# pps-lab/rofl-project-code

Measured on NVIDIA B200. Metric: range-proved commitment elements/s (prove & verify), higher is better.
Workload: dtype u32 (8 saturated 32-bit limbs of GF(2^255-19), IMAD.WIDE.U32 with 64-bit accumulate; scalars mod l)

## Files before the change

### rofl-project-code_b200/csrc/engine.cuh

```cuda
#pragma once
#include "kernels.cuh"
#include "rt.cuh"
#include <map>
#include <mutex>
#include <shared_mutex>
#include <condition_variable>
#include <thread>
#include <atomic>
#ifndef ROFL_EMUL
#include <sys/resource.h>
#endif
#include <algorithm>
#include <chrono>
#include <cstdio>

enum { ROFL_ERR_BITSIZE_ = -7 };
enum { DOM_RANGE_PROVE = 1, DOM_RANGE_VERIFY = 2, DOM_SQUARE = 3, DOM_L2_PROVE = 4, DOM_L2_VERIFY = 5, DOM_CRP = 6, DOM_RND_VEC = 7, DOM_RANDPROOF = 8, DOM_SQUARE_RAND = 9,
       DOM_CRP_BATCH = 0x62707263 ,
       DOM_SQ_RLC = 0x6c727173 ,
       DOM_RP_RLC = 0x6c727072 ,
       DOM_SRP_RLC = 0x6c727273  };
enum { PROF_FOLD = 0, PROF_MSM = 1, PROF_COMMIT = 2, PROF_SQUARE = 3, PROF_RTMSM = 4, PROF_TAIL = 5, PROF_FRZ = 6, PROF_SLOTS = 8 };

struct gens_entry { int n = 0; int cap = 0; niels_st *G = nullptr, *H = nullptr;
// ... 161 lines not shown
static inline void engine_destroy(rofl_engine &e) {
    for (lane *l : e.lanes) { for (int g = 0; g < ROFL_MAX_GROUPS; g++) { rt_sync(l->q[g].hi); rt_sync(l->q[g].lo); rt_sync(l->side[g]); } lane_delete(l); }
    e.lanes.clear();
    for (auto &pp : e.pins) rt_host_free(pp.first);
    e.pins.clear();
    std::lock_guard<std::mutex> lk(g_shared_mu);
    dev_shared *sh = e.sh; e.sh = nullptr;
    if (!sh || --sh->refs > 0) return;
    rt_raw_free(sh->tabB); rt_raw_free(sh->tabH);
    for (auto &g : sh->gens) { rt_raw_free(g.second.G); rt_raw_free(g.second.H); rt_raw_free(g.second.RTG); rt_raw_free(g.second.RTH); }
    for (auto &b : sh->bsgs) { rt_raw_free(b.second.keys); rt_raw_free(b.second.vals); }
    g_shared.erase(sh->device); delete sh;
    rt_trim();
}
static inline gens_entry engine_gens(rofl_engine &e, tables_use &tu, cudaStream_t s, int n, int m) {
    dev_shared &sh = *e.sh;
    for (;;) {
        auto it = sh.gens.find(n);
        if (it != sh.gens.end() && it->second.cap >= m) return it->second;
        tu.upgrade();
        gens_entry &g = sh.gens[n];
        if (g.cap >= m) continue;
        int newcap = std::max(m, g.cap * 2);
        niels_st *G = (niels_st *)rt_raw_malloc(sizeof(niels_st) * (size_t)n * newcap);
        niels_st *H = (niels_st *)rt_raw_malloc(sizeof(niels_st) * (size_t)n * newcap);
        if (g.cap) { rt_d2d(G, g.G, sizeof(niels_st) * (size_t)n * g.cap, s); rt_d2d(H, g.H, sizeof(niels_st) * (size_t)n * g.cap, s); }
        int cnt = 2 * (newcap - g.cap);
        LAUNCH(k_gens_build, dim3((cnt + 63) / 64), dim3(64), s, G, H, n, g.cap, newcap);
        rt_sync(s);
        rt_raw_free(g.G); rt_raw_free(g.H);
        g.n = n; g.cap = newcap; g.G = G; g.H = H;
    }
}
static inline void rt_fill(rt_tables &t, int c) { t.c = c; t.nw = msm_nw(c); t.B = 1 << (c - 1); msm_recode_const(t.K, c); }
static inline size_t rt_table_bytes(size_t cnt, int c) { return 2 * cnt * (size_t)msm_nw(c) * ((size_t)1 << (c - 1)) * sizeof(niels_st); }
static inline bool engine_rt(rofl_engine &e, tables_use &tu, cudaStream_t s, int n, int m, rt_tables &out) {
    if (!e.use_rt) return false;
    dev_shared &sh = *e.sh;
    for (;;) {
        gens_entry &g = sh.gens[n];
        if (g.rt_cap >= m) { g.last_use = ++sh.clock; out.G = g.RTG; out.H = g.RTH; rt_fill(out, g.rt_c); return true; }
        if (g.rt_nofit && m >= g.rt_nofit) return false;
        if (!tu.excl) { tu.upgrade(); continue; }
        const size_t cnt = (size_t)n * m;
        if ((double)rt_table_bytes(cnt, 8) > 170e9) { g.rt_nofit = m; return false; }
        rt_sync(s); rt_raw_free(g.RTG); rt_raw_free(g.RTH); g.RTG = g.RTH = nullptr; g.rt_cap = 0; g.rt_bytes = 0;
        rt_trim();
        const int want = std::max(8, std::min(RT_MAX_BITS, e.rt_bits));
        int c = 0;
        for (;;) {
            const size_t have = rt_free_mem();
            for (c = want; c >= 8; c--) if ((double)(rt_table_bytes(cnt, c) + cnt * msm_nw(c) * sizeof(p3_st)) <= e.rt_mem_frac * (double)have) break;
            if (c == want) break;
            gens_entry *victim = nullptr;
            for (auto &kv : sh.gens) if (&kv.second != &g && kv.second.RTG && (!victim || kv.second.last_use < victim->last_use)) victim = &kv.second;
            if (!victim) break;
            rt_raw_free(victim->RTG); rt_raw_free(victim->RTH); victim->RTG = victim->RTH = nullptr; victim->rt_cap = 0; victim->rt_bytes = 0;
        }
        if (c < 8) { g.rt_nofit = m; sh.free_hint = rt_free_mem(); return false; }
        rt_tables t; rt_fill(t, c);
        const size_t bytes = cnt * rt_row_entries(t) * sizeof(niels_st);
        niels_st *RTG = (niels_st *)rt_raw_malloc(bytes), *RTH = (niels_st *)rt_raw_malloc(bytes);
        {
            dev_buf P(cnt * t.nw * sizeof(p3_st), s);
            const size_t rows = cnt * t.nw, thr = rows * (t.B / 16);
            for (int which = 0; which < 2; which++) {
                LAUNCH(k_rt_shifts, dim3((unsigned)((cnt + 127) / 128)), dim3(128), s, P.as<p3_st>(), which ? g.H : g.G, (uint32_t)cnt, t.c, t.nw);
                LAUNCH(k_rt_rows, dim3((unsigned)((thr + 127) / 128)), dim3(128), s, which ? RTH : RTG, P.as<p3_st>(), rows, t.B);
            }
            rt_sync(s);
        }
        g.RTG = RTG; g.RTH = RTH; g.rt_cap = m; g.rt_c = c; g.rt_bytes = 2 * bytes;
        rt_trim();
        sh.free_hint = rt_free_mem();
    }
}
static inline void engine_drop_rt(rofl_engine &e) {
    std::unique_lock<std::shared_mutex> ex(e.sh->tab_mu);
    for (auto &g : e.sh->gens) { rt_raw_free(g.second.RTG); rt_raw_free(g.second.RTH); g.second.RTG = g.second.RTH = nullptr; g.second.rt_cap = 0; g.second.rt_bytes = 0; g.second.rt_nofit = 0; }
}
static inline int rt_blocks(size_t T, int C, int per_max = 0) {
    const size_t slots = 148 * RTM_BLOCKS, max_nb = std::max<size_t>(1, (T + 127) / 128);
    if (per_max > 0) {
        const size_t nb = std::min(max_nb, (T + 128 * (size_t)per_max - 1) / (128 * (size_t)per_max));
        return (int)std::max<size_t>(1, nb);
// ... 17 lines not shown
struct msm_plan { int c, nw; uint32_t slices, slice_len; bool big = false; uint32_t parts = 1; size_t out_count(size_t n_msm) const { return n_msm * slices * (size_t)nw; } };
static inline int msm_pick_c(size_t T) {
    int best = 8; double bc = 1e300;
    for (int c = 3; c <= 8; c++) { const double B = (double)(1 << (c - 1)), cost = (double)msm_nw(c) * ((double)T + B * c); if (cost < bc) { bc = cost; best = c; } }
    return best;
}
static inline size_t bm_min_terms() { static const size_t v = getenv("ROFL_BM_MIN") ? (size_t)atoll(getenv("ROFL_BM_MIN")) : (size_t)32768; return v; }
static inline msm_plan msm_plan_forced(size_t T, int c, int knob) {
    msm_plan p; p.c = std::max(3, std::min(16, c)); p.nw = msm_nw(p.c); p.slices = 1; p.slice_len = (uint32_t)T;
    if (p.c > 8) { p.big = true; p.parts = (uint32_t)std::max(1, std::min(8, knob)); return p; }
    if (T > 0) { p.slices = (uint32_t)std::max<size_t>(1, std::min<size_t>(std::max(knob, 1), T)); p.slice_len = (uint32_t)((T + p.slices - 1) / p.slices); p.slices = (uint32_t)((T + p.slice_len - 1) / p.slice_len); }
    return p;
}
static inline msm_plan msm_plan_for(size_t T, size_t n_msm, size_t big_min = 0) {
    msm_plan p; p.c = msm_pick_c(T); p.slices = 1; p.slice_len = (uint32_t)T;
    if (const char *fc = getenv("ROFL_MSM_C"))
        return msm_plan_forced(T, atoi(fc), getenv("ROFL_MSM_SLICES") ? atoi(getenv("ROFL_MSM_SLICES")) : 1);
    if (T >= (big_min ? big_min : bm_min_terms())) {
        p.big = true; p.c = std::max(9, std::min(16, ilog2_sz(T + 1) - 6)); p.nw = msm_nw(p.c);
        const size_t threads = n_msm * (size_t)p.nw * ((size_t)1 << (p.c - 1));
        p.parts = (uint32_t)std::max<size_t>(1, std::min<size_t>(8, (148 * 1024 + threads - 1) / threads));
        return p;
    }
    const size_t wpb = MSM_THREADS >> (p.c - 1), blocks = n_msm * ((msm_nw(p.c) + wpb - 1) / wpb), slots = 148 * 4;
    if (blocks < slots && T >= 4096) {
        p.slices = (uint32_t)std::min<size_t>((slots + blocks - 1) / blocks, T / 2048);
        p.slice_len = (uint32_t)((T + p.slices - 1) / p.slices); p.slices = (uint32_t)((T + p.slice_len - 1) / p.slice_len);
        p.c = msm_pick_c(p.slice_len);
    }
    p.nw = msm_nw(p.c);
    return p;
}
static inline void run_msm(rofl_engine &e, cudaStream_t s, msm_args a, const msm_plan &p, uint32_t n_msm) {
    a.c = p.c; a.nw = p.nw; a.slices = p.slices; a.slice_len = p.slice_len; msm_recode_const(a.K, p.c);
    void *tk = rt_prof_begin(PROF_MSM, s);
    if (p.big) {
        const size_t B = (size_t)1 << (p.c - 1), nslot = (size_t)n_msm * p.nw * (B + 1);
        dev_buf d_start(4 * nslot, s), d_cur(4 * nslot, s), d_sorted(4 * (size_t)n_msm * p.nw * a.T, s), d_bkt(sizeof(p3_st) * (size_t)n_msm * p.nw * B * p.parts, s);
        a.bm_start = d_start.as<uint32_t>(); a.bm_cur = d_cur.as<uint32_t>(); a.bm_sorted = d_sorted.as<uint32_t>(); a.bm_bkt = d_bkt.as<p3_st>(); a.parts = p.parts;
        a.top_bits = (uint32_t)(254 - p.c * (p.nw - 1)); a.parts_top = 0;
        if ((int)a.top_bits < p.c - 4) a.parts_top = (uint32_t)((B * p.parts) >> (a.top_bits + 1));
        rt_memset(d_start.p, 0, 4 * nslot, s);
        const dim3 gt((unsigned)((a.T + 255) / 256), n_msm);
        LAUNCH(k_bm_hist, gt, dim3(256), s, a, 0);
        LAUNCH_COOP(k_bm_scan, dim3(p.nw, n_msm), dim3(256), s, a);
        LAUNCH(k_bm_hist, gt, dim3(256), s, a, 1);
        LAUNCH(k_bm_accum, dim3((unsigned)(((size_t)p.nw * B * p.parts + 127) / 128), n_msm), dim3(128), s, a);
        LAUNCH_COOP(k_bm_reduce, dim3(p.nw, n_msm), dim3(128), s, a);
    } else {
        const int wpb = MSM_THREADS >> (p.c - 1);
        LAUNCH_COOP(k_msm, dim3((p.nw + wpb - 1) / wpb, n_msm, p.slices), dim3(MSM_THREADS), s, a);
    }
    rt_prof_end(PROF_MSM, tk, s);
}
static inline msm_seg mk_seg(const void *base, uint32_t count, uint32_t stride, int kind, uint32_t np = 0, int hi = 0) { msm_seg s; s.base = base; s.count = count; s.stride = stride; s.kind = kind; s.np = np; s.hi = hi; return s; }
static inline void run_finalize(cudaStream_t s, const finalize_args &f) { LAUNCH_COOP(k_finalize, dim3(f.count), dim3(FIN_THREADS), s, f); }
static inline void fin_windows(finalize_args &f, const p3_st *win, const msm_plan &p) { f.windows = win; f.c = p.c; f.nw = p.nw; f.slices = p.slices; }


static void absorb_commitments(rofl_engine &e, cudaStream_t s, transcript *d_ts, const uint8_t *d_V32, int label_id, int n, int m, int C) {
    if (m <= e.ts_host_m) {
        ts_absorb_args aa = {}; aa.ts = d_ts; aa.V32 = d_V32; aa.m = (uint32_t)m; aa.n = (uint32_t)n; aa.label_id = label_id;
        LAUNCH_COOP(k_ts_absorbV, dim3(C), dim3(TS_THREADS), s, aa);
        return;
    }
    std::vector<uint8_t> hV(32 * (size_t)C * m); std::vector<transcript> ts(C);
    rt_d2h(hV.data(), d_V32, hV.size(), s); rt_sync(s);
// ... 1022 lines not shown
```

### rofl-project-code_b200/csrc/fe25519.cuh

```cuda
#pragma once
#include <stdint.h>
#include <string.h>

#if defined(__CUDACC__)
#define HD __host__ __device__ __forceinline__
#define HDNI static __host__ __device__ __noinline__
#else
#define HD inline
#define HDNI static inline
#endif
#define FE_ASSERT(c) ((void)0)
#ifndef FE_MUL_ROWS
#define FE_MUL_ROWS 1
#endif
#ifndef FE_INLINE_MUL
#define FE_INLINE_MUL 1
#endif
#if defined(__CUDACC__) && !FE_INLINE_MUL
#define HDMUL static __host__ __device__ __noinline__
#elif defined(__CUDACC__)
#define HDMUL __host__ __device__ __forceinline__
#else
#define HDMUL inline
#endif

#if !defined(__CUDACC__)
struct alignas(16) uint4 { uint32_t x, y, z, w; };
static inline uint4 make_uint4(uint32_t x, uint32_t y, uint32_t z, uint32_t w) { uint4 r; r.x = x; r.y = y; r.z = z; r.w = w; return r; }
#define __align__(n) alignas(n)
#endif

#define FE_LIMBS 8
struct fe { uint32_t v[8]; };

HD void fe_0(fe &h) { for (int i = 0; i < 8; i++) h.v[i] = 0; }
HD void fe_1(fe &h) { fe_0(h); h.v[0] = 1; }
HD void fe_carry(fe &h, const fe &f) { h = f; }

HD void fe_add(fe &h, const fe &f, const fe &g) {
#if defined(__CUDA_ARCH__)
    uint32_t r0, r1, r2, r3, r4, r5, r6, r7, c;
    asm("add.cc.u32 %0, %9, %17;\n\taddc.cc.u32 %1, %10, %18;\n\taddc.cc.u32 %2, %11, %19;\n\taddc.cc.u32 %3, %12, %20;\n\t"
        "addc.cc.u32 %4, %13, %21;\n\taddc.cc.u32 %5, %14, %22;\n\taddc.cc.u32 %6, %15, %23;\n\taddc.cc.u32 %7, %16, %24;\n\taddc.u32 %8, 0, 0;"
        : "=&r"(r0), "=&r"(r1), "=&r"(r2), "=&r"(r3), "=&r"(r4), "=&r"(r5), "=&r"(r6), "=&r"(r7), "=&r"(c)
        : "r"(f.v[0]), "r"(f.v[1]), "r"(f.v[2]), "r"(f.v[3]), "r"(f.v[4]), "r"(f.v[5]), "r"(f.v[6]), "r"(f.v[7]),
          "r"(g.v[0]), "r"(g.v[1]), "r"(g.v[2]), "r"(g.v[3]), "r"(g.v[4]), "r"(g.v[5]), "r"(g.v[6]), "r"(g.v[7]));
    c *= 38;
    asm("add.cc.u32 %0, %0, %8;\n\taddc.cc.u32 %1, %1, 0;\n\taddc.cc.u32 %2, %2, 0;\n\taddc.cc.u32 %3, %3, 0;\n\t"
        "addc.cc.u32 %4, %4, 0;\n\taddc.cc.u32 %5, %5, 0;\n\taddc.cc.u32 %6, %6, 0;\n\taddc.cc.u32 %7, %7, 0;\n\taddc.u32 %8, 0, 0;"
        : "+r"(r0), "+r"(r1), "+r"(r2), "+r"(r3), "+r"(r4), "+r"(r5), "+r"(r6), "+r"(r7), "+r"(c));
    r0 += 38 * c;
    h.v[0] = r0; h.v[1] = r1; h.v[2] = r2; h.v[3] = r3; h.v[4] = r4; h.v[5] = r5; h.v[6] = r6; h.v[7] = r7;
#else
    uint64_t c = 0; uint32_t r[8];
    for (int i = 0; i < 8; i++) { c += (uint64_t)f.v[i] + g.v[i]; r[i] = (uint32_t)c; c >>= 32; }
    c *= 38;
    for (int i = 0; i < 8; i++) { c += r[i]; r[i] = (uint32_t)c; c >>= 32; }
    r[0] += 38 * (uint32_t)c;
    for (int i = 0; i < 8; i++) h.v[i] = r[i];
#endif
}
HD void fe_sub(fe &h, const fe &f, const fe &g) {
#if defined(__CUDA_ARCH__)
    uint32_t r0, r1, r2, r3, r4, r5, r6, r7, b;
    asm("sub.cc.u32 %0, %9, %17;\n\tsubc.cc.u32 %1, %10, %18;\n\tsubc.cc.u32 %2, %11, %19;\n\tsubc.cc.u32 %3, %12, %20;\n\t"
        "subc.cc.u32 %4, %13, %21;\n\tsubc.cc.u32 %5, %14, %22;\n\tsubc.cc.u32 %6, %15, %23;\n\tsubc.cc.u32 %7, %16, %24;\n\tsubc.u32 %8, 0, 0;"
        : "=&r"(r0), "=&r"(r1), "=&r"(r2), "=&r"(r3), "=&r"(r4), "=&r"(r5), "=&r"(r6), "=&r"(r7), "=&r"(b)
        : "r"(f.v[0]), "r"(f.v[1]), "r"(f.v[2]), "r"(f.v[3]), "r"(f.v[4]), "r"(f.v[5]), "r"(f.v[6]), "r"(f.v[7]),
          "r"(g.v[0]), "r"(g.v[1]), "r"(g.v[2]), "r"(g.v[3]), "r"(g.v[4]), "r"(g.v[5]), "r"(g.v[6]), "r"(g.v[7]));
    b = (b & 1) * 38;
    asm("sub.cc.u32 %0, %0, %8;\n\tsubc.cc.u32 %1, %1, 0;\n\tsubc.cc.u32 %2, %2, 0;\n\tsubc.cc.u32 %3, %3, 0;\n\t"
        "subc.cc.u32 %4, %4, 0;\n\tsubc.cc.u32 %5, %5, 0;\n\tsubc.cc.u32 %6, %6, 0;\n\tsubc.cc.u32 %7, %7, 0;\n\tsubc.u32 %8, 0, 0;"
        : "+r"(r0), "+r"(r1), "+r"(r2), "+r"(r3), "+r"(r4), "+r"(r5), "+r"(r6), "+r"(r7), "+r"(b));
    r0 -= 38 * (b & 1);
    h.v[0] = r0; h.v[1] = r1; h.v[2] = r2; h.v[3] = r3; h.v[4] = r4; h.v[5] = r5; h.v[6] = r6; h.v[7] = r7;
#else
    int64_t c = 0; uint32_t r[8];
    for (int i = 0; i < 8; i++) { c += (int64_t)f.v[i] - (int64_t)g.v[i]; r[i] = (uint32_t)c; c >>= 32; }
    c *= 38;
    for (int i = 0; i < 8; i++) { c += r[i]; r[i] = (uint32_t)c; c >>= 32; }
    r[0] -= 38 * (uint32_t)(-c);
    for (int i = 0; i < 8; i++) h.v[i] = r[i];
#endif
}
HD void fe_sub4(fe &h, const fe &f, const fe &g) { fe_sub(h, f, g); }
HD void fe_neg(fe &h, const fe &f) { fe z; fe_0(z); fe_sub(h, z, f); }

#if defined(__CUDA_ARCH__)
__device__ __forceinline__ uint64_t fe_mad_wide(uint32_t a, uint32_t b, uint32_t c) {
    uint64_t d; asm("mad.wide.u32 %0, %1, %2, %3;" : "=l"(d) : "r"(a), "r"(b), "l"((uint64_t)c)); return d;
}
__device__ __forceinline__ void fe_reduce512(fe &h, const uint32_t t[16]) {
    uint64_t d0 = fe_mad_wide(t[8], 38, t[0]), d1 = fe_mad_wide(t[9], 38, t[1]), d2 = fe_mad_wide(t[10], 38, t[2]), d3 = fe_mad_wide(t[11], 38, t[3]);
    uint64_t d4 = fe_mad_wide(t[12], 38, t[4]), d5 = fe_mad_wide(t[13], 38, t[5]), d6 = fe_mad_wide(t[14], 38, t[6]), d7 = fe_mad_wide(t[15], 38, t[7]);
    uint32_t r0 = (uint32_t)d0, r1, r2, r3, r4, r5, r6, r7, top;
    asm("add.cc.u32 %0, %8, %9;\n\taddc.cc.u32 %1, %10, %11;\n\taddc.cc.u32 %2, %12, %13;\n\taddc.cc.u32 %3, %14, %15;\n\t"
        "addc.cc.u32 %4, %16, %17;\n\taddc.cc.u32 %5, %18, %19;\n\taddc.cc.u32 %6, %20, %21;\n\taddc.u32 %7, %22, 0;"
        : "=&r"(r1), "=&r"(r2), "=&r"(r3), "=&r"(r4), "=&r"(r5), "=&r"(r6), "=&r"(r7), "=&r"(top)
        : "r"((uint32_t)d1), "r"((uint32_t)(d0 >> 32)), "r"((uint32_t)d2), "r"((uint32_t)(d1 >> 32)), "r"((uint32_t)d3), "r"((uint32_t)(d2 >> 32)),
          "r"((uint32_t)d4), "r"((uint32_t)(d3 >> 32)), "r"((uint32_t)d5), "r"((uint32_t)(d4 >> 32)), "r"((uint32_t)d6), "r"((uint32_t)(d5 >> 32)),
          "r"((uint32_t)d7), "r"((uint32_t)(d6 >> 32)), "r"((uint32_t)(d7 >> 32)));
    uint32_t c = top * 38;
    asm("add.cc.u32 %0, %0, %8;\n\taddc.cc.u32 %1, %1, 0;\n\taddc.cc.u32 %2, %2, 0;\n\taddc.cc.u32 %3, %3, 0;\n\t"
        "addc.cc.u32 %4, %4, 0;\n\taddc.cc.u32 %5, %5, 0;\n\taddc.cc.u32 %6, %6, 0;\n\taddc.cc.u32 %7, %7, 0;\n\taddc.u32 %8, 0, 0;"
        : "+r"(r0), "+r"(r1), "+r"(r2), "+r"(r3), "+r"(r4), "+r"(r5), "+r"(r6), "+r"(r7), "+r"(c));
    r0 += 38 * c;
    h.v[0] = r0; h.v[1] = r1; h.v[2] = r2; h.v[3] = r3; h.v[4] = r4; h.v[5] = r5; h.v[6] = r6; h.v[7] = r7;
}
#define FE_MAC(lo, hi, ex, a, b) asm("mad.lo.cc.u32 %0, %3, %4, %0;\n\tmadc.hi.cc.u32 %1, %3, %4, %1;\n\taddc.u32 %2, %2, 0;" : "+r"(lo), "+r"(hi), "+r"(ex) : "r"(a), "r"(b))
#define FE_MUL0(lo, hi, a, b) do { uint64_t p_; asm("mul.wide.u32 %0, %1, %2;" : "=l"(p_) : "r"(a), "r"(b)); lo = (uint32_t)p_; hi = (uint32_t)(p_ >> 32); } while (0)
__device__ __forceinline__ void fe_columns_to_words(uint32_t t[16], const uint32_t lo[15], const uint32_t hi[15], const uint32_t ex[15]) {
    t[0] = lo[0];
    asm("add.cc.u32 %0, %15, %30;\n\taddc.cc.u32 %1, %16, %31;\n\taddc.cc.u32 %2, %17, %32;\n\taddc.cc.u32 %3, %18, %33;\n\taddc.cc.u32 %4, %19, %34;\n\t"
        "addc.cc.u32 %5, %20, %35;\n\taddc.cc.u32 %6, %21, %36;\n\taddc.cc.u32 %7, %22, %37;\n\taddc.cc.u32 %8, %23, %38;\n\taddc.cc.u32 %9, %24, %39;\n\t"
        "addc.cc.u32 %10, %25, %40;\n\taddc.cc.u32 %11, %26, %41;\n\taddc.cc.u32 %12, %27, %42;\n\taddc.cc.u32 %13, %28, %43;\n\taddc.u32 %14, %29, 0;"
        : "=&r"(t[1]), "=&r"(t[2]), "=&r"(t[3]), "=&r"(t[4]), "=&r"(t[5]), "=&r"(t[6]), "=&r"(t[7]), "=&r"(t[8]), "=&r"(t[9]), "=&r"(t[10]), "=&r"(t[11]), "=&r"(t[12]), "=&r"(t[13]), "=&r"(t[14]), "=&r"(t[15])
        : "r"(lo[1]), "r"(lo[2]), "r"(lo[3]), "r"(lo[4]), "r"(lo[5]), "r"(lo[6]), "r"(lo[7]), "r"(lo[8]), "r"(lo[9]), "r"(lo[10]), "r"(lo[11]), "r"(lo[12]), "r"(lo[13]), "r"(lo[14]), "r"(hi[14]),
          "r"(hi[0]), "r"(hi[1]), "r"(hi[2]), "r"(hi[3]), "r"(hi[4]), "r"(hi[5]), "r"(hi[6]), "r"(hi[7]), "r"(hi[8]), "r"(hi[9]), "r"(hi[10]), "r"(hi[11]), "r"(hi[12]), "r"(hi[13]));
    asm("add.cc.u32 %0, %0, %14;\n\taddc.cc.u32 %1, %1, %15;\n\taddc.cc.u32 %2, %2, %16;\n\taddc.cc.u32 %3, %3, %17;\n\taddc.cc.u32 %4, %4, %18;\n\t"
        "addc.cc.u32 %5, %5, %19;\n\taddc.cc.u32 %6, %6, %20;\n\taddc.cc.u32 %7, %7, %21;\n\taddc.cc.u32 %8, %8, %22;\n\taddc.cc.u32 %9, %9, %23;\n\t"
        "addc.cc.u32 %10, %10, %24;\n\taddc.cc.u32 %11, %11, %25;\n\taddc.cc.u32 %12, %12, %26;\n\taddc.u32 %13, %13, %27;"
        : "+r"(t[2]), "+r"(t[3]), "+r"(t[4]), "+r"(t[5]), "+r"(t[6]), "+r"(t[7]), "+r"(t[8]), "+r"(t[9]), "+r"(t[10]), "+r"(t[11]), "+r"(t[12]), "+r"(t[13]), "+r"(t[14]), "+r"(t[15])
        : "r"(ex[0]), "r"(ex[1]), "r"(ex[2]), "r"(ex[3]), "r"(ex[4]), "r"(ex[5]), "r"(ex[6]), "r"(ex[7]), "r"(ex[8]), "r"(ex[9]), "r"(ex[10]), "r"(ex[11]), "r"(ex[12]), "r"(ex[13]));
}
__device__ __forceinline__ void fe_mul_rows(uint32_t t[16], const fe &f, const fe &g) {
    uint32_t e[16], o[17];
    for (int k = 0; k < 16; k++) e[k] = 0;
    for (int k = 0; k < 17; k++) o[k] = 0;
    FE_MUL0(e[0], e[1], f.v[0], g.v[0]);
    FE_MUL0(e[2], e[3], f.v[0], g.v[2]);
    FE_MUL0(e[4], e[5], f.v[0], g.v[4]);
    FE_MUL0(e[6], e[7], f.v[0], g.v[6]);
    FE_MUL0(o[1], o[2], f.v[0], g.v[1]);
    FE_MUL0(o[3], o[4], f.v[0], g.v[3]);
    FE_MUL0(o[5], o[6], f.v[0], g.v[5]);
    FE_MUL0(o[7], o[8], f.v[0], g.v[7]);
    asm("mad.lo.cc.u32 %0, %8, %9, %0;\n\tmadc.hi.cc.u32 %1, %8, %9, %1;\n\tmadc.lo.cc.u32 %2, %8, %10, %2;\n\tmadc.hi.cc.u32 %3, %8, %10, %3;\n\tmadc.lo.cc.u32 %4, %8, %11, %4;\n\tmadc.hi.cc.u32 %5, %8, %11, %5;\n\tmadc.lo.cc.u32 %6, %8, %12, %6;\n\tmadc.hi.u32 %7, %8, %12, %7;"
        : "+r"(e[2]), "+r"(e[3]), "+r"(e[4]), "+r"(e[5]), "+r"(e[6]), "+r"(e[7]), "+r"(e[8]), "+r"(e[9])
        : "r"(f.v[1]), "r"(g.v[1]), "r"(g.v[3]), "r"(g.v[5]), "r"(g.v[7]));
    asm("mad.lo.cc.u32 %0, %9, %10, %0;\n\tmadc.hi.cc.u32 %1, %9, %10, %1;\n\tmadc.lo.cc.u32 %2, %9, %11, %2;\n\tmadc.hi.cc.u32 %3, %9, %11, %3;\n\tmadc.lo.cc.u32 %4, %9, %12, %4;\n\tmadc.hi.cc.u32 %5, %9, %12, %5;\n\tmadc.lo.cc.u32 %6, %9, %13, %6;\n\tmadc.hi.cc.u32 %7, %9, %13, %7;\n\taddc.u32 %8, 0, 0;"
        : "+r"(o[1]), "+r"(o[2]), "+r"(o[3]), "+r"(o[4]), "+r"(o[5]), "+r"(o[6]), "+r"(o[7]), "+r"(o[8]), "+r"(o[9])
// ... 215 lines not shown
```

### rofl-project-code_b200/csrc/kernels.cuh

```cuda
#pragma once
#include "devfn.cuh"

#include "rt.cuh"
#ifndef ROFL_EMUL
#define KERNEL extern "C" __global__
#define LB(t, b) __launch_bounds__(t, b)
#define DEV __device__ __forceinline__
#define KLAUNCH(k, coop, PARAMS, ARGS) void launch_##k(dim3 g_, dim3 b_, cudaStream_t s_, KL_UNPACK PARAMS) { rt_host_timer t_(&rt_host_prof::launch, #k); void *tl_ = rt_timeline_begin(#k, s_, g_.x * g_.y * g_.z); k<<<g_, b_, 0, s_>>> ARGS; rt_check(cudaGetLastError(), #k); rt_timeline_end(tl_, s_); rt_count_launch(#k); }
#else
#define KERNEL static
#define LB(t, b)
#define DEV inline
#define KLAUNCH(k, coop, PARAMS, ARGS) void launch_##k(dim3 g_, dim3 b_, cudaStream_t s_, KL_UNPACK PARAMS) { (void)s_; emu_launch(g_, b_, coop, [&] { k ARGS; }); }
#endif
#define KL_UNPACK(...) __VA_ARGS__
#if defined(KG_ALL)
#define KG_TABLES 1
#define KG_COMMIT 1
#define KG_SCALAR 1
#define KG_MSM 1
#define KG_FOLD 1
#define KG_SQUARE 1
#define KG_BSGS 1
#define KG_TS 1
// ... 218 lines not shown

#ifdef KG_MSM
KERNEL void LB(128, 2) k_bits_sum(p3_st *partial, const uint64_t *vals, const niels_st *G, const niels_st *H, int n, int m) {
    __shared__ p3_st buf[128];
    int c = blockIdx.y, tid = threadIdx.x;
    size_t N = (size_t)n * m;
    ge_p3 acc; ge_p3_0(acc);
    for (size_t k = (size_t)blockIdx.x * blockDim.x + tid; k < N; k += (size_t)gridDim.x * blockDim.x) {
        size_t j = k / n; int i = (int)(k % n);
        bool bit = (vals[(size_t)c * m + j] >> i) & 1;
        acc_add_niels(acc, (bit ? G : H) + k, !bit);
    }
    block_sum_p3(acc, buf, tid, blockDim.x);
    if (tid == 0) st_p3(partial + (size_t)c * gridDim.x + blockIdx.x, acc);
}
KLAUNCH(k_bits_sum, true, (p3_st *partial, const uint64_t *vals, const niels_st *G, const niels_st *H, int n, int m), (partial, vals, G, H, n, m))
#endif

#define MSM_THREADS 128
#define MSM_SORT 8192
#define MSM_MAXW 85
struct msm_seg { const void *base; uint32_t count; uint32_t stride; int kind; uint32_t np; int hi; };
struct msm_var { const sc_st *scalars; msm_seg seg[4]; };
struct msm_args {
    msm_var v[2]; uint32_t split;
    int nseg; uint32_t T, scalar_stride;
    int c, nw; uint32_t K[9];
    uint32_t slices, slice_len;
    p3_st *out;
    uint32_t *bm_start, *bm_cur, *bm_sorted; p3_st *bm_bkt; uint32_t parts;
    uint32_t top_bits, parts_top;
};
HD int msm_nw(int c) { return (254 + c - 1) / c; }
HD void msm_recode_const(uint32_t K[9], int c) {
    for (int i = 0; i < 9; i++) K[i] = 0;
    const uint32_t bm1 = (1u << (c - 1)) - 1; const int nw = msm_nw(c);
    for (int w = 0; w < nw; w++) { int bit = c * w; uint64_t v = (uint64_t)bm1 << (bit & 31); K[bit >> 5] |= (uint32_t)v; if ((bit >> 5) + 1 < 9) K[(bit >> 5) + 1] |= (uint32_t)(v >> 32); }
}
HD void msm_recode(uint32_t xk[9], const sc &x, const uint32_t K[9]) {
    uint64_t cy = 0;
    for (int i = 0; i < 8; i++) { cy += (uint64_t)x.v[i] + K[i]; xk[i] = (uint32_t)cy; cy >>= 32; }
    xk[8] = (uint32_t)cy + K[8];
}
HD int msm_digit(const uint32_t xk[9], int w, int c) {
    int bit = c * w, i = bit >> 5, sh = bit & 31;
    uint64_t v = (uint64_t)xk[i] | ((uint64_t)(i + 1 < 9 ? xk[i + 1] : 0) << 32);
    return (int)((v >> sh) & ((1u << c) - 1)) - ((1 << (c - 1)) - 1);
}
HD void msm_add_term(ge_p3 &acc, const msm_var &v, int nseg, uint32_t idx, uint32_t t, bool neg) {
    uint32_t start = 0; const void *base = nullptr; size_t rec = 0; int kind = -1;
    for (int s = 0; s < nseg; s++) {
        const msm_seg &g = v.seg[s];
        const bool here = kind < 0 && t < start + g.count;
        if (here) { const uint32_t q = t - start, j = g.np ? (q / g.np) * 2 * g.np + (g.hi ? g.np : 0) + q % g.np : q; base = g.base; rec = (size_t)idx * g.stride + j; kind = g.kind; }
        start += g.count;
    }
    if (kind == 0) acc_add_niels(acc, (const niels_st *)base + rec, neg);
    else if (kind == 1) acc_add_p3(acc, (const p3_st *)base + rec, neg);
}
#ifdef KG_MSM
KERNEL void LB(MSM_THREADS, 4) k_msm(msm_args a) {
    __shared__ uint16_t sorted[MSM_SORT];
    __shared__ int cnt[MSM_THREADS], off[MSM_THREADS + 1], cur[MSM_THREADS];
    __shared__ p3_st bk[MSM_THREADS];
    const int tid = threadIdx.x, c = a.c, B = 1 << (c - 1), wpb = MSM_THREADS / B;
    const int w0 = blockIdx.x * wpb, wl_mine = tid / B, b_mine = tid & (B - 1);
    const uint32_t msm = blockIdx.y, slice = blockIdx.z;
    const msm_var &v = msm < a.split ? a.v[0] : a.v[1];
    const uint32_t idx = msm < a.split ? msm : msm - a.split;
// ... 875 lines not shown
void launch_k_ipp_fold_points(dim3 g_, dim3 b_, cudaStream_t s_, fold_args a);
void launch_k_decompress_batch(dim3 g_, dim3 b_, cudaStream_t s_, p3_st *out, uint8_t *out32, const uint8_t *in, size_t D, size_t Dp, size_t K, const p3_st *offset, int *bad);
void launch_k_decompress(dim3 g_, dim3 b_, cudaStream_t s_, p3_st *out, uint8_t *out32, const uint8_t *in, size_t count_in, size_t count_out, const p3_st *offset, int *bad, size_t bad_group);
void launch_k_verify_tables(dim3 g_, dim3 b_, cudaStream_t s_, sc_st *tab, vtab_layout t, sc_st *var, uint32_t var_stride, const sc_st *chal, int chal_stride, const sc_st *yinvpow2, const sc_st *zpow2, int m);
void launch_k_verify_scalars(dim3 g_, dim3 b_, cudaStream_t s_, sc_st *gh, const sc_st *tab, vtab_layout t, const sc_st *chal, int chal_stride, int n, int C);
void launch_k_square_prove(dim3 g_, dim3 b_, cudaStream_t s_, square_args a);
void launch_k_sigma_prove(dim3 g_, dim3 b_, cudaStream_t s_, sigma_args a);
void launch_k_sigma_verify(dim3 g_, dim3 b_, cudaStream_t s_, int kind, const uint8_t *proofs, const uint8_t *commits, size_t D, const niels_st *tabB, const niels_st *tabH, int *result, size_t group);
void launch_k_sigma_rlc_prep(dim3 g_, dim3 b_, cudaStream_t s_, sigma_rlc_args a);
void launch_k_sigma_rlc_scalars(dim3 g_, dim3 b_, cudaStream_t s_, sigma_rlc_args a);
void launch_k_sigma_rlc_points(dim3 g_, dim3 b_, cudaStream_t s_, sigma_rlc_args a);
void launch_k_square_verify(dim3 g_, dim3 b_, cudaStream_t s_, const uint8_t *proofs, const uint8_t *commits, size_t D, const niels_st *tabB, const niels_st *tabH, int *result, size_t group);
void launch_k_hash_tree(dim3 g_, dim3 b_, cudaStream_t s_, uint8_t *out, const uint8_t *in, size_t n);
void launch_k_aggregate(dim3 g_, dim3 b_, cudaStream_t s_, uint8_t *out, const uint8_t *pts, size_t n_clients, size_t D, int init_base, int *bad);
void launch_k_bsgs_build(dim3 g_, dim3 b_, cudaStream_t s_, unsigned long long *keys, uint32_t *vals, uint32_t cap, uint32_t m, const niels_st *tabB, int *distinct);
void launch_k_bsgs_solve(dim3 g_, dim3 b_, cudaStream_t s_, uint8_t *out_sc, float *out_f32, const uint8_t *pts, size_t D, const unsigned long long *keys, const uint32_t *vals, uint32_t cap, uint32_t m, uint64_t size, uint64_t max_it, int bsgs_bits, int n_bits, int frac, const niels_st *tabB, int *flags);
void launch_k_f32_to_scalar(dim3 g_, dim3 b_, cudaStream_t s_, uint8_t *out, const float *v, size_t D, int n_bits, int frac, int *flags);
void launch_k_scalar_to_f32(dim3 g_, dim3 b_, cudaStream_t s_, float *out, const uint8_t *in, size_t D, int n_bits, int frac);
void launch_k_l2_sums(dim3 g_, dim3 b_, cudaStream_t s_, sc_st *partial, const float *v, const uint8_t *blind, size_t D, int n_bits, int frac, int *flags);
void launch_k_join96(dim3 g_, dim3 b_, cudaStream_t s_, uint8_t *out96, const uint8_t *pairs64, const uint8_t *sq64, size_t D);
void launch_k_validate_points(dim3 g_, dim3 b_, cudaStream_t s_, const uint8_t *rec, size_t stride, size_t offset, size_t D, int *bad, size_t group);
void launch_k_split96(dim3 g_, dim3 b_, cudaStream_t s_, uint8_t *L, uint8_t *sq64, uint8_t *csq, const uint8_t *in96, size_t D);
void launch_k_points_sum(dim3 g_, dim3 b_, cudaStream_t s_, p3_st *partial, const uint8_t *pts32, size_t D, int *bad);
void launch_k_crp_sums(dim3 g_, dim3 b_, cudaStream_t s_, sc_st *partial, const float *v, const uint8_t *blind, size_t D, int n_bits, int frac, pow_tab ctab, int *flags);
void launch_k_crp_pows(dim3 g_, dim3 b_, cudaStream_t s_, sc_st *out, size_t D, pow_tab ctab);
void launch_k_pairs_join(dim3 g_, dim3 b_, cudaStream_t s_, uint8_t *pairs, const uint8_t *L, const uint8_t *R, size_t D);
void launch_k_pairs_split(dim3 g_, dim3 b_, cudaStream_t s_, uint8_t *L, uint8_t *R, const uint8_t *pairs, size_t D);
void launch_k_pairs_gather_L(dim3 g_, dim3 b_, cudaStream_t s_, uint8_t *out, const uint8_t *pairs, size_t D, size_t num, size_t K);
void launch_k_crp_batch_points(dim3 g_, dim3 b_, cudaStream_t s_, p3_st *P, const uint8_t *pairs, const uint8_t *cp, size_t D, uint32_t G, int *bad);
void launch_k_crp_batch_scalars(dim3 g_, dim3 b_, cudaStream_t s_, sc_st *s, size_t D, uint32_t G, pow_tab ctab, const sc_st *rho);

#define RT_MAXW 32
#define RT_MAX_BITS 11
struct rt_tables { const niels_st *G, *H; int c, nw, B; uint32_t K[9]; };
HD size_t rt_row_entries(const rt_tables &t) { return (size_t)t.nw * t.B; }
#ifdef KG_TABLES
KERNEL void LB(128, 2) k_rt_shifts(p3_st *P, const niels_st *gens, uint32_t count, int c, int nw) {
    uint32_t j = blockIdx.x * blockDim.x + threadIdx.x;
    if (j >= count) return;
    ge_niels g; ld_niels(g, gens + j);
    ge_p3 p; ge_niels_to_p3(p, g);
    for (int w = 0; w < nw; w++) {
        st_p3(P + (size_t)j * nw + w, p);
        for (int k = 0; k < c; k++) ge_p3_dbl(p, p);
    }
}
KLAUNCH(k_rt_shifts, false, (p3_st *P, const niels_st *gens, uint32_t count, int c, int nw), (P, gens, count, c, nw))
KERNEL void LB(128, 2) k_rt_rows(niels_st *RT, const p3_st *P, size_t rows, int B) {
    const int gpr = B / 16;
    size_t idx = (size_t)blockIdx.x * blockDim.x + threadIdx.x;
    if (idx >= rows * gpr) return;
    size_t row = idx / gpr; int grp = (int)(idx % gpr);
    ge_p3 base; ld_p3(base, P + row);
    ge_cached cb; ge_p3_to_cached(cb, base);
    ge_p3 cur; ge_p3_0(cur);
    { uint32_t k = 16 * grp + 1; for (int b = 9; b >= 0; b--) { ge_p3_dbl(cur, cur); if ((k >> b) & 1) ge_add_cached(cur, cur, cb); } }
    ge_p3 pts[16]; fe pre[16], acc; fe_1(acc);
    for (int e = 0; e < 16; e++) { pts[e] = cur; pre[e] = acc; fe_mul(acc, acc, cur.Z); if (e < 15) ge_add_cached(cur, cur, cb); }
    fe inv; fe_invert(inv, acc);
    for (int e = 15; e >= 0; e--) {
        fe zinv; fe_mul(zinv, inv, pre[e]); fe_mul(inv, inv, pts[e].Z);
        ge_niels n; ge_p3_to_niels(n, pts[e], zinv);
        st_niels(RT + row * B + 16 * grp + e, n);
    }
}
KLAUNCH(k_rt_rows, false, (niels_st *RT, const p3_st *P, size_t rows, int B), (RT, P, rows, B))
#endif

HD void rt_digits(int16_t d[RT_MAXW], const sc &x, const rt_tables &t) {
    uint32_t xk[9]; msm_recode(xk, x, t.K);
    for (int w = 0; w < t.nw; w++) d[w] = (int16_t)msm_digit(xk, w, t.c);
}
HD void rt_mul_acc(ge_p3 &acc, const niels_st *row0, const sc &x, const rt_tables &t) {
    uint32_t xk[9]; msm_recode(xk, x, t.K);
    for (int w = 0; w < t.nw; w++) {
        const int dw = msm_digit(xk, w, t.c);
        if (dw != 0) acc_add_niels(acc, row0 + (size_t)w * t.B + (dw > 0 ? dw : -dw) - 1, dw < 0);
    }
}
struct rt_msm_args { const sc_st *scalars; uint32_t T, scalar_stride, nG, np; int mode; rt_tables rt; p3_st *partial; };
#ifndef RTM_STAGES
#define RTM_STAGES 3
#endif
#ifndef RTM_BLOCKS
#define RTM_BLOCKS 4
#endif
#ifdef ROFL_EMUL
DEV void cp_async16(void *dst, const void *src) { *(uint4 *)dst = *(const uint4 *)src; }
DEV void cp_async_commit() {}
template <int N> DEV void cp_async_wait() {}
#else
DEV void cp_async16(void *dst, const void *src) { asm volatile("cp.async.cg.shared.global [%0], [%1], 16;" ::"r"((uint32_t)__cvta_generic_to_shared(dst)), "l"(src) : "memory"); }
DEV void cp_async_commit() { asm volatile("cp.async.commit_group;" ::: "memory"); }
template <int N> DEV void cp_async_wait() { asm volatile("cp.async.wait_group %0;" ::"n"(N) : "memory"); }
#endif
struct rtm_stage { uint4 rec[RTM_STAGES][6][128]; uint4 scal[2][2][128]; };
struct rtm_cursor { uint32_t xk[9]; const niels_st *row0; uint32_t term, w, flags; };
DEV void rtm_consume(ge_p3 &acc, const rtm_stage &sm, uint32_t slot, int tid, bool neg) {
    const uint4 *q = &sm.rec[slot][0][tid]; const uint32_t op = neg ? 256u : 0u, om = neg ? 0u : 256u;
    uint4 v0 = q[op], v1 = q[op + 128], v2 = q[om], v3 = q[om + 128], v4 = q[512], v5 = q[640];
    ge_niels m;
    m.yplusx.v[0] = v0.x; m.yplusx.v[1] = v0.y; m.yplusx.v[2] = v0.z; m.yplusx.v[3] = v0.w; m.yplusx.v[4] = v1.x; m.yplusx.v[5] = v1.y; m.yplusx.v[6] = v1.z; m.yplusx.v[7] = v1.w;
    m.yminusx.v[0] = v2.x; m.yminusx.v[1] = v2.y; m.yminusx.v[2] = v2.z; m.yminusx.v[3] = v2.w; m.yminusx.v[4] = v3.x; m.yminusx.v[5] = v3.y; m.yminusx.v[6] = v3.z; m.yminusx.v[7] = v3.w;
    m.xy2d.v[0] = v4.x; m.xy2d.v[1] = v4.y; m.xy2d.v[2] = v4.z; m.xy2d.v[3] = v4.w; m.xy2d.v[4] = v5.x; m.xy2d.v[5] = v5.y; m.xy2d.v[6] = v5.z; m.xy2d.v[7] = v5.w;
    ge_p1p1 t; ge_madd_p1p1(t, acc, m);
    fe z = t.Z; fe_cmov(t.Z, t.T, neg); fe_cmov(t.T, z, neg);
    ge_p1p1_to_p3(acc, t);
}
#ifdef KG_MSM
DEV void rtm_produce(rtm_cursor &p, rtm_stage &sm, const rt_msm_args &a, const sc_st *scal, uint32_t t0, uint32_t stride, uint32_t nterm, uint32_t g, uint32_t total, uint32_t slot, int tid) {
    if (g < total) {
        if (p.w == (uint32_t)a.rt.nw) {
// ... 526 lines not shown
```

Before: 1.616 million.

## Trim precomputed table windows and replace multiply-by-38 with shift-add reduction

Sizes the precomputed-table window count for 253-bit scalars instead of 254, which can drop one window row per generator and so shrinks table memory and per-term additions. Recoding constants now take the window count explicitly. Field reduction of the high 256 bits replaces the mad.wide-by-38 products with three funnel-shifted add chains (x<<1 + x<<2 + x<<5), and the carry multiply-by-38 becomes a mask. Unused rt_digits and rt_mul_acc helpers are removed. The shift-add chains issue more integer instructions than the multiply version, and the reduced window count assumes scalars below 2^253, which holds for scalars mod l.

```diff
diff --git a/rofl-project-code_b200/csrc/engine.cuh b/rofl-project-code_b200/csrc/engine.cuh
--- a/rofl-project-code_b200/csrc/engine.cuh
+++ b/rofl-project-code_b200/csrc/engine.cuh
@@ -217,8 +217,8 @@
         g.n = n; g.cap = newcap; g.G = G; g.H = H;
     }
 }
-static inline void rt_fill(rt_tables &t, int c) { t.c = c; t.nw = msm_nw(c); t.B = 1 << (c - 1); msm_recode_const(t.K, c); }
-static inline size_t rt_table_bytes(size_t cnt, int c) { return 2 * cnt * (size_t)msm_nw(c) * ((size_t)1 << (c - 1)) * sizeof(niels_st); }
+static inline void rt_fill(rt_tables &t, int c) { t.c = c; t.nw = rt_nw(c); t.B = 1 << (c - 1); msm_recode_const(t.K, c, t.nw); }
+static inline size_t rt_table_bytes(size_t cnt, int c) { return 2 * cnt * (size_t)rt_nw(c) * ((size_t)1 << (c - 1)) * sizeof(niels_st); }
 static inline bool engine_rt(rofl_engine &e, tables_use &tu, cudaStream_t s, int n, int m, rt_tables &out) {
     if (!e.use_rt) return false;
     dev_shared &sh = *e.sh;
@@ -235,7 +235,7 @@
         int c = 0;
         for (;;) {
             const size_t have = rt_free_mem();
-            for (c = want; c >= 8; c--) if ((double)(rt_table_bytes(cnt, c) + cnt * msm_nw(c) * sizeof(p3_st)) <= e.rt_mem_frac * (double)have) break;
+            for (c = want; c >= 8; c--) if ((double)(rt_table_bytes(cnt, c) + cnt * rt_nw(c) * sizeof(p3_st)) <= e.rt_mem_frac * (double)have) break;
             if (c == want) break;
             gens_entry *victim = nullptr;
             for (auto &kv : sh.gens) if (&kv.second != &g && kv.second.RTG && (!victim || kv.second.last_use < victim->last_use)) victim = &kv.second;
@@ -319,7 +319,7 @@
     return p;
 }
 static inline void run_msm(rofl_engine &e, cudaStream_t s, msm_args a, const msm_plan &p, uint32_t n_msm) {
-    a.c = p.c; a.nw = p.nw; a.slices = p.slices; a.slice_len = p.slice_len; msm_recode_const(a.K, p.c);
+    a.c = p.c; a.nw = p.nw; a.slices = p.slices; a.slice_len = p.slice_len; msm_recode_const(a.K, p.c, p.nw);
     void *tk = rt_prof_begin(PROF_MSM, s);
     if (p.big) {
         const size_t B = (size_t)1 << (p.c - 1), nslot = (size_t)n_msm * p.nw * (B + 1);
diff --git a/rofl-project-code_b200/csrc/fe25519.cuh b/rofl-project-code_b200/csrc/fe25519.cuh
--- a/rofl-project-code_b200/csrc/fe25519.cuh
+++ b/rofl-project-code_b200/csrc/fe25519.cuh
@@ -37,6 +37,9 @@
 HD void fe_1(fe &h) { fe_0(h); h.v[0] = 1; }
 HD void fe_carry(fe &h, const fe &f) { h = f; }
 
+#if defined(__CUDA_ARCH__)
+__device__ __forceinline__ uint32_t fe_38_if(uint32_t c) { return (0u - c) & 38u; }
+#endif
 HD void fe_add(fe &h, const fe &f, const fe &g) {
 #if defined(__CUDA_ARCH__)
     uint32_t r0, r1, r2, r3, r4, r5, r6, r7, c;
@@ -45,11 +48,11 @@
         : "=&r"(r0), "=&r"(r1), "=&r"(r2), "=&r"(r3), "=&r"(r4), "=&r"(r5), "=&r"(r6), "=&r"(r7), "=&r"(c)
         : "r"(f.v[0]), "r"(f.v[1]), "r"(f.v[2]), "r"(f.v[3]), "r"(f.v[4]), "r"(f.v[5]), "r"(f.v[6]), "r"(f.v[7]),
           "r"(g.v[0]), "r"(g.v[1]), "r"(g.v[2]), "r"(g.v[3]), "r"(g.v[4]), "r"(g.v[5]), "r"(g.v[6]), "r"(g.v[7]));
-    c *= 38;
+    c = fe_38_if(c);
     asm("add.cc.u32 %0, %0, %8;\n\taddc.cc.u32 %1, %1, 0;\n\taddc.cc.u32 %2, %2, 0;\n\taddc.cc.u32 %3, %3, 0;\n\t"
         "addc.cc.u32 %4, %4, 0;\n\taddc.cc.u32 %5, %5, 0;\n\taddc.cc.u32 %6, %6, 0;\n\taddc.cc.u32 %7, %7, 0;\n\taddc.u32 %8, 0, 0;"
         : "+r"(r0), "+r"(r1), "+r"(r2), "+r"(r3), "+r"(r4), "+r"(r5), "+r"(r6), "+r"(r7), "+r"(c));
-    r0 += 38 * c;
+    r0 += fe_38_if(c);
     h.v[0] = r0; h.v[1] = r1; h.v[2] = r2; h.v[3] = r3; h.v[4] = r4; h.v[5] = r5; h.v[6] = r6; h.v[7] = r7;
 #else
     uint64_t c = 0; uint32_t r[8];
@@ -68,11 +71,11 @@
         : "=&r"(r0), "=&r"(r1), "=&r"(r2), "=&r"(r3), "=&r"(r4), "=&r"(r5), "=&r"(r6), "=&r"(r7), "=&r"(b)
         : "r"(f.v[0]), "r"(f.v[1]), "r"(f.v[2]), "r"(f.v[3]), "r"(f.v[4]), "r"(f.v[5]), "r"(f.v[6]), "r"(f.v[7]),
           "r"(g.v[0]), "r"(g.v[1]), "r"(g.v[2]), "r"(g.v[3]), "r"(g.v[4]), "r"(g.v[5]), "r"(g.v[6]), "r"(g.v[7]));
-    b = (b & 1) * 38;
+    b &= 38;
     asm("sub.cc.u32 %0, %0, %8;\n\tsubc.cc.u32 %1, %1, 0;\n\tsubc.cc.u32 %2, %2, 0;\n\tsubc.cc.u32 %3, %3, 0;\n\t"
         "subc.cc.u32 %4, %4, 0;\n\tsubc.cc.u32 %5, %5, 0;\n\tsubc.cc.u32 %6, %6, 0;\n\tsubc.cc.u32 %7, %7, 0;\n\tsubc.u32 %8, 0, 0;"
         : "+r"(r0), "+r"(r1), "+r"(r2), "+r"(r3), "+r"(r4), "+r"(r5), "+r"(r6), "+r"(r7), "+r"(b));
-    r0 -= 38 * (b & 1);
+    r0 -= b & 38;
     h.v[0] = r0; h.v[1] = r1; h.v[2] = r2; h.v[3] = r3; h.v[4] = r4; h.v[5] = r5; h.v[6] = r6; h.v[7] = r7;
 #else
     int64_t c = 0; uint32_t r[8];
@@ -87,26 +90,29 @@
 HD void fe_neg(fe &h, const fe &f) { fe z; fe_0(z); fe_sub(h, z, f); }
 
 #if defined(__CUDA_ARCH__)
-__device__ __forceinline__ uint64_t fe_mad_wide(uint32_t a, uint32_t b, uint32_t c) {
-    uint64_t d; asm("mad.wide.u32 %0, %1, %2, %3;" : "=l"(d) : "r"(a), "r"(b), "l"((uint64_t)c)); return d;
-}
+#define FE_ADD_SHL(s, x) do {                                                                                                            \
+    const uint32_t w0_ = (x)[0] << (s), w1_ = __funnelshift_l((x)[0], (x)[1], s), w2_ = __funnelshift_l((x)[1], (x)[2], s),             \
+                   w3_ = __funnelshift_l((x)[2], (x)[3], s), w4_ = __funnelshift_l((x)[3], (x)[4], s), w5_ = __funnelshift_l((x)[4], (x)[5], s), \
+                   w6_ = __funnelshift_l((x)[5], (x)[6], s), w7_ = __funnelshift_l((x)[6], (x)[7], s), w8_ = (x)[7] >> (32 - (s));             \
+    asm("add.cc.u32 %0, %0, %9;\n\taddc.cc.u32 %1, %1, %10;\n\taddc.cc.u32 %2, %2, %11;\n\taddc.cc.u32 %3, %3, %12;\n\t"                   \
+        "addc.cc.u32 %4, %4, %13;\n\taddc.cc.u32 %5, %5, %14;\n\taddc.cc.u32 %6, %6, %15;\n\taddc.cc.u32 %7, %7, %16;\n\taddc.u32 %8, %8, %17;" \
+        : "+r"(r0), "+r"(r1), "+r"(r2), "+r"(r3), "+r"(r4), "+r"(r5), "+r"(r6), "+r"(r7), "+r"(top)                                     \
+        : "r"(w0_), "r"(w1_), "r"(w2_), "r"(w3_), "r"(w4_), "r"(w5_), "r"(w6_), "r"(w7_), "r"(w8_));                                      \
+} while (0)
 __device__ __forceinline__ void fe_reduce512(fe &h, const uint32_t t[16]) {
-    uint64_t d0 = fe_mad_wide(t[8], 38, t[0]), d1 = fe_mad_wide(t[9], 38, t[1]), d2 = fe_mad_wide(t[10], 38, t[2]), d3 = fe_mad_wide(t[11], 38, t[3]);
-    uint64_t d4 = fe_mad_wide(t[12], 38, t[4]), d5 = fe_mad_wide(t[13], 38, t[5]), d6 = fe_mad_wide(t[14], 38, t[6]), d7 = fe_mad_wide(t[15], 38, t[7]);
-    uint32_t r0 = (uint32_t)d0, r1, r2, r3, r4, r5, r6, r7, top;
-    asm("add.cc.u32 %0, %8, %9;\n\taddc.cc.u32 %1, %10, %11;\n\taddc.cc.u32 %2, %12, %13;\n\taddc.cc.u32 %3, %14, %15;\n\t"
-        "addc.cc.u32 %4, %16, %17;\n\taddc.cc.u32 %5, %18, %19;\n\taddc.cc.u32 %6, %20, %21;\n\taddc.u32 %7, %22, 0;"
-        : "=&r"(r1), "=&r"(r2), "=&r"(r3), "=&r"(r4), "=&r"(r5), "=&r"(r6), "=&r"(r7), "=&r"(top)
-        : "r"((uint32_t)d1), "r"((uint32_t)(d0 >> 32)), "r"((uint32_t)d2), "r"((uint32_t)(d1 >> 32)), "r"((uint32_t)d3), "r"((uint32_t)(d2 >> 32)),
-          "r"((uint32_t)d4), "r"((uint32_t)(d3 >> 32)), "r"((uint32_t)d5), "r"((uint32_t)(d4 >> 32)), "r"((uint32_t)d6), "r"((uint32_t)(d5 >> 32)),
-          "r"((uint32_t)d7), "r"((uint32_t)(d6 >> 32)), "r"((uint32_t)(d7 >> 32)));
-    uint32_t c = top * 38;
+    const uint32_t *hi = t + 8;
+    uint32_t r0 = t[0], r1 = t[1], r2 = t[2], r3 = t[3], r4 = t[4], r5 = t[5], r6 = t[6], r7 = t[7], top = 0;
+    FE_ADD_SHL(1, hi);
+    FE_ADD_SHL(2, hi);
+    FE_ADD_SHL(5, hi);
+    uint32_t c = (top << 5) + (top << 2) + (top << 1);
     asm("add.cc.u32 %0, %0, %8;\n\taddc.cc.u32 %1, %1, 0;\n\taddc.cc.u32 %2, %2, 0;\n\taddc.cc.u32 %3, %3, 0;\n\t"
         "addc.cc.u32 %4, %4, 0;\n\taddc.cc.u32 %5, %5, 0;\n\taddc.cc.u32 %6, %6, 0;\n\taddc.cc.u32 %7, %7, 0;\n\taddc.u32 %8, 0, 0;"
         : "+r"(r0), "+r"(r1), "+r"(r2), "+r"(r3), "+r"(r4), "+r"(r5), "+r"(r6), "+r"(r7), "+r"(c));
-    r0 += 38 * c;
+    r0 += fe_38_if(c);
     h.v[0] = r0; h.v[1] = r1; h.v[2] = r2; h.v[3] = r3; h.v[4] = r4; h.v[5] = r5; h.v[6] = r6; h.v[7] = r7;
 }
+#undef FE_ADD_SHL
 #define FE_MAC(lo, hi, ex, a, b) asm("mad.lo.cc.u32 %0, %3, %4, %0;\n\tmadc.hi.cc.u32 %1, %3, %4, %1;\n\taddc.u32 %2, %2, 0;" : "+r"(lo), "+r"(hi), "+r"(ex) : "r"(a), "r"(b))
 #define FE_MUL0(lo, hi, a, b) do { uint64_t p_; asm("mul.wide.u32 %0, %1, %2;" : "=l"(p_) : "r"(a), "r"(b)); lo = (uint32_t)p_; hi = (uint32_t)(p_ >> 32); } while (0)
 __device__ __forceinline__ void fe_columns_to_words(uint32_t t[16], const uint32_t lo[15], const uint32_t hi[15], const uint32_t ex[15]) {
diff --git a/rofl-project-code_b200/csrc/kernels.cuh b/rofl-project-code_b200/csrc/kernels.cuh
--- a/rofl-project-code_b200/csrc/kernels.cuh
+++ b/rofl-project-code_b200/csrc/kernels.cuh
@@ -274,9 +274,9 @@
     uint32_t top_bits, parts_top;
 };
 HD int msm_nw(int c) { return (254 + c - 1) / c; }
-HD void msm_recode_const(uint32_t K[9], int c) {
+HD void msm_recode_const(uint32_t K[9], int c, int nw) {
     for (int i = 0; i < 9; i++) K[i] = 0;
-    const uint32_t bm1 = (1u << (c - 1)) - 1; const int nw = msm_nw(c);
+    const uint32_t bm1 = (1u << (c - 1)) - 1;
     for (int w = 0; w < nw; w++) { int bit = c * w; uint64_t v = (uint64_t)bm1 << (bit & 31); K[bit >> 5] |= (uint32_t)v; if ((bit >> 5) + 1 < 9) K[(bit >> 5) + 1] |= (uint32_t)(v >> 32); }
 }
 HD void msm_recode(uint32_t xk[9], const sc &x, const uint32_t K[9]) {
@@ -1218,6 +1218,7 @@
 
 #define RT_MAXW 32
 #define RT_MAX_BITS 11
+HD int rt_nw(int c) { return (253 + c - 1) / c; }
 struct rt_tables { const niels_st *G, *H; int c, nw, B; uint32_t K[9]; };
 HD size_t rt_row_entries(const rt_tables &t) { return (size_t)t.nw * t.B; }
 #ifdef KG_TABLES
@@ -1253,17 +1254,6 @@
 KLAUNCH(k_rt_rows, false, (niels_st *RT, const p3_st *P, size_t rows, int B), (RT, P, rows, B))
 #endif
 
-HD void rt_digits(int16_t d[RT_MAXW], const sc &x, const rt_tables &t) {
-    uint32_t xk[9]; msm_recode(xk, x, t.K);
-    for (int w = 0; w < t.nw; w++) d[w] = (int16_t)msm_digit(xk, w, t.c);
-}
-HD void rt_mul_acc(ge_p3 &acc, const niels_st *row0, const sc &x, const rt_tables &t) {
-    uint32_t xk[9]; msm_recode(xk, x, t.K);
-    for (int w = 0; w < t.nw; w++) {
-        const int dw = msm_digit(xk, w, t.c);
-        if (dw != 0) acc_add_niels(acc, row0 + (size_t)w * t.B + (dw > 0 ? dw : -dw) - 1, dw < 0);
-    }
-}
 struct rt_msm_args { const sc_st *scalars; uint32_t T, scalar_stride, nG, np; int mode; rt_tables rt; p3_st *partial; };
 #ifndef RTM_STAGES
 #define RTM_STAGES 3
```

Result: slower. 1.509 million, median of 6 (-6.6%).
